# Brockaaa/scenery-insitu

Hardware: AMD Instinct MI355X
Metric: frames/sec @1920x1080 (8x512^3 volume) (higher is better)
Workload: dtype f32

## Files before the change

scenery-insitu_amd/csrc/insitu_hip.cpp:

```cpp
#include "insitu_host.h"

#include <cmath>
#include <cstdio>
#include <algorithm>
#include <cstdlib>
#include <cstring>
#include <limits>
#include <string>
#include <vector>

#pragma clang fp contract(off)

namespace {

thread_local std::string g_create_error;

size_t dtype_size(int dt) { return dt == INSITU_U8 ? 1 : (dt == INSITU_U16 ? 2 : 4); }

}

int fail(insitu_ctx* c, int code, const std::string& msg) {
    if (c) c->err = msg;
    else g_create_error = msg;
    return code;
// ... 37 lines not shown
    f.h_ctr_pending = false;
    f.h_ctr_valid = true;
    if (!c->cache_adaptive || f.h_ctr->march_rays == 0) return;
    const unsigned long long want = f.h_ctr->cache_cursor + f.h_ctr->cache_cursor / 4;
    const size_t to = std::min((size_t)want, c->cache_max_chunks);
    if (to > f.cache_chunks) f.cache_grow_to = (uint32_t)to;
}

hipError_t cache_realloc(FrameSlot& f, size_t chunks) {
    f.cache_chunks = 0;
    const hipError_t e = f.cache.try_alloc(chunks * 8);
    if (e == hipSuccess) f.cache_chunks = (uint32_t)chunks;
    return e;
}

}

int check_fault(insitu_ctx* c, FrameSlot& f) {
    cache_observe(c, f);
    if (!f.counters || !f.search_launched) return 0;
    uint32_t fault = 0;
    if (f.h_ctr_valid) fault = f.h_ctr->fault;
    else if (hipMemcpy(&fault, &f.counters->fault, sizeof fault, hipMemcpyDeviceToHost) != hipSuccess) fault = 1;
    if (fault) return fail(c, -6, "VDI search kernel exceeded its loop bound (internal error)");
    return 0;
}

namespace {

float4* cvdi_col(const insitu_ctx* c) { return c->rank == 0 ? c->d_gvdi_col : c->d_cvdi_col; }
float2* cvdi_dep(const insitu_ctx* c) { return c->rank == 0 ? c->d_gvdi_dep : c->d_cvdi_dep; }
uint16_t* cvdi_cnt(const insitu_ctx* c) { return c->rank == 0 ? c->d_gvdi_cnt : c->d_cvdi_cnt; }

void record(FrameSlot& f, FrameEvent i, hipStream_t s) {
    if (hipEventRecord(f.ev[i], s) == hipSuccess) f.ev_valid[i] = true;
}

hipError_t compact_enqueue(insitu_ctx* c, FrameSlot& f, hipStream_t s) {
    record(f, EvCompactStart, s);
    hipError_t e = hipMemsetAsync(c->d_cursor, 0, sizeof(uint32_t) * (size_t)c->N, s);
    if (e != hipSuccess) return e;
    CompactParams cp{};
    cp.col = f.vcol_send;
    cp.dep = f.vdep_send;
    cp.pend = f.seg_pending;
    cp.pend_stride = (size_t)c->W * (size_t)c->H;
    cp.W = c->W; cp.H = c->H; cp.S = c->S; cp.B = c->BV; cp.nstrips = c->N; cp.strip_w = c->strip_w;
    cp.strip_tiles = c->strip_tiles; cp.ytiles = (c->H + 7) / 8; cp.skip_d = c->rank;
    cp.blockE = c->blockE;
    cp.out_col = c->d_ccol_send;
    cp.out_dep = c->d_cdep_send;
    cp.out_meta = c->d_meta_send;
    cp.meta_bytes = c->meta_bytes;
    cp.cursor = c->d_cursor;
    e = launch_vdi_compact(cp, s);
    if (e == hipSuccess) record(f, EvCompactEnd, s);
    return e;
}

hipError_t wait_peer_reads(insitu_ctx* c, hipStream_t s) {
    if (!c->group) return hipSuccess;
    for (const insitu_ctx* q : c->group->ranks) {
        if (!q || q == c || !q->cur->ev_valid[EvPeerReadsDone]) continue;
        hipError_t e = hipStreamWaitEvent(s, q->cur->ev[EvPeerReadsDone], 0);
        if (e != hipSuccess) return e;
    }
    return hipSuccess;
}

int create_slot_events(insitu_ctx* c, FrameSlot& f) {
    for (auto& ev : f.ev)
        if (!ev && hipEventCreate(&ev) != hipSuccess) return fail(c, -3, "hipEventCreate failed");
    return 0;
}

int alloc_slot(insitu_ctx* c, FrameSlot& f, size_t chunks) {
    int rc = 0;
    if ((rc = create_slot_events(c, f))) return rc;
    const size_t sendE = (size_t)c->N * (size_t)c->BV * c->blockE;
    const size_t px = (size_t)c->BV * (size_t)c->W * (size_t)c->H;
    if ((rc = f.vcol_send.alloc(c, sendE)) || (rc = f.vdep_send.alloc(c, sendE))) return rc;
    const size_t oct = (size_t)c->BV * (size_t)c->S * (size_t)c->ncx * (size_t)c->ncy;
    if ((rc = f.octree.alloc(c, oct ? oct : 1))) return rc;
    if ((rc = f.seg_pending.alloc(c, px)) || (rc = f.seg_steps.alloc(c, sendE))) return rc;
    if (hipMemset(f.seg_pending, 0, sizeof(uint16_t) * px) != hipSuccess)
        return fail(c, -3, "hipMemset of the supersegment counts failed");
    if (c->cfg.keep_passes && (rc = f.passes.alloc(c, px))) return rc;
    if ((rc = f.counters.alloc(c, 1))) return rc;
    if (hipMemset(f.counters, 0, sizeof(GenCounters)) != hipSuccess)
        return fail(c, -3, "hipMemset of the generator counters failed");
    if (chunks == 0) return 0;
    if ((rc = f.cache.alloc(c, chunks * 8)) || (rc = f.queue.alloc(c, (size_t)c->B * (size_t)c->W * (size_t)c->H)))
        return rc;
    if (f.h_ctr.try_alloc(1) != hipSuccess) return fail(c, -5, "hipHostMalloc of the generator counters failed");
    std::memset(f.h_ctr, 0, sizeof(GenCounters));
    f.cache_chunks = (uint32_t)chunks;
    const size_t ntile = (size_t)c->B * (size_t)((c->H + 7) / 8) * (size_t)c->N * (size_t)c->strip_tiles;
    if (ntile < ((size_t)1 << 24)) {
        size_t tb = 0;
        if (sort_tiles_desc(nullptr, tb, nullptr, nullptr, nullptr, nullptr, (int)ntile, nullptr) != hipSuccess)
            return fail(c, -3, "hipcub radix sort: temporary storage query failed");
        if ((rc = f.tile_keys.alloc(c, 2 * ntile)) || (rc = f.tile_ids.alloc(c, 2 * ntile)) ||
            (rc = f.sort_tmp.alloc(c, tb + 1)))
            return rc;
        c->sort_tmp_bytes = tb;
    }
    return 0;
}

size_t padded_tiles(const insitu_ctx* c, int sup) {
    return (size_t)c->B * (size_t)((((c->H + 7) / 8) + sup - 1) / sup * sup) *
           (size_t)((c->N * c->strip_tiles + sup - 1) / sup * sup);
}

}

extern "C" {

int insitu_abi_version(void) { return INSITU_ABI_VERSION; }

int insitu_local_group_create(int nranks, insitu_local_group** out) {
    if (!out || nranks < 1 || nranks > kMaxLists) return fail(nullptr, -1, "insitu_local_group_create: bad arguments");
    *out = new insitu_local_group();
    (*out)->ranks.assign((size_t)nranks, nullptr);
    return 0;
}

void insitu_local_group_destroy(insitu_local_group* g) { delete g; }

int insitu_comm_id(void* out, size_t cap) {
    if (!out || cap < sizeof(ncclUniqueId)) return fail(nullptr, -1, "insitu_comm_id: buffer too small");
    ncclUniqueId id;
    ncclResult_t r = ncclGetUniqueId(&id);
    if (r != ncclSuccess) return fail(nullptr, -4, std::string("ncclGetUniqueId: ") + ncclGetErrorString(r));
    std::memcpy(out, &id, sizeof id);
    return 0;
}

const char* insitu_last_error(const insitu_ctx* ctx) { return ctx ? ctx->err.c_str() : g_create_error.c_str(); }

int insitu_create(const insitu_config* cfg, insitu_ctx** out) {
    if (!cfg || !out) return fail(nullptr, -1, "insitu_create: null argument");
    *out = nullptr;
    const insitu_config& k = *cfg;
    if (k.nranks < 1 || k.rank < 0 || k.rank >= k.nranks) return fail(nullptr, -1, "insitu_create: bad rank/nranks");
    if (k.width <= 0 || k.height <= 0) return fail(nullptr, -1, "insitu_create: bad window size");
    if (k.mode != INSITU_MODE_VDI && k.mode != INSITU_MODE_PLAIN) return fail(nullptr, -1, "insitu_create: bad mode");
    if (k.bricks_per_rank < 1 || k.bricks_per_rank > kMaxBricks)
        return fail(nullptr, -1, "insitu_create: bricks_per_rank must be in [1," + std::to_string(kMaxBricks) + "]");
    if (k.nranks * k.bricks_per_rank > kMaxLists)
        return fail(nullptr, -1, "insitu_create: nranks*bricks_per_rank exceeds " + std::to_string(kMaxLists));
    if (k.mode == INSITU_MODE_VDI && (k.max_supersegments < 1 || k.max_supersegments > 255))
        return fail(nullptr, -1, "insitu_create: max_supersegments must be in [1,255]");
    if (k.mode == INSITU_MODE_VDI && k.width % k.nranks != 0)
        return fail(nullptr, -1, "insitu_create: width must divide evenly into nranks screen strips");
    if (k.mode == INSITU_MODE_PLAIN && k.height % k.nranks != 0)
        return fail(nullptr, -1, "insitu_create: height (texture dim1) must divide evenly into nranks strips");
    if (k.nranks > 1 && !k.comm_id && !k.local_group)
        return fail(nullptr, -1, "insitu_create: comm_id (or local_group) required when nranks > 1");
    if (k.local_group && ((int)k.local_group->ranks.size() != k.nranks || k.local_group->ranks[k.rank]))
        return fail(nullptr, -1, "insitu_create: local_group size differs from nranks, or rank already taken");
    if (k.composite_vdi && k.mode != INSITU_MODE_VDI)
        return fail(nullptr, -1, "insitu_create: composite_vdi needs VDI mode");
    if (k.merge_bricks && k.mode != INSITU_MODE_VDI)
        return fail(nullptr, -1, "insitu_create: merge_bricks needs VDI mode");
    if (k.max_output_supersegments < 0 || k.max_output_supersegments > 255)
        return fail(nullptr, -1, "insitu_create: max_output_supersegments must be in [0,255]");
// ... 366 lines not shown
        std::memcpy(iv, cam->inv_view, sizeof iv);
        std::memcpy(ip, cam->inv_proj, sizeof ip);
    } else if (!mat4_inverse(cam->view, iv) || !mat4_inverse(cam->proj, ip)) {
        return fail(c, -1, "insitu_set_camera: view or projection matrix is singular");
    }
    mat4_mul_f(iv, ip, m->ipv);
    mat4_mul_f(cam->proj, cam->view, m->pv);
    std::memcpy(m->view, cam->view, sizeof m->view);
    m->nw = cam->nw; m->fwnw = cam->fwnw; m->tmax = cam->tmax;
    return 0;
}

void set_slot_camera(insitu_ctx* c, FrameSlot& f, const FrameCamera& m) {
    std::memcpy(f.ipv, m.ipv, sizeof f.ipv);
    std::memcpy(f.pv, m.pv, sizeof f.pv);
    std::memcpy(f.view, m.view, sizeof f.view);
    c->camera_set = true;
}

int render_check(insitu_ctx* c, const insitu_camera* cam, FrameCamera* m) {
    if (!cam) return fail(c, -1, "insitu_render: null camera");
    if (!c->d_tf) return fail(c, -1, "insitu_render: transfer function not set");
    for (int b = 0; b < c->B; ++b) {
        if (!c->bricks[b].valid) return fail(c, -1, "insitu_render: brick slot " + std::to_string(b) + " not set");
        if (c->bricks[b].dtype != c->bricks[0].dtype)
            return fail(c, -1, "insitu_render: all bricks of a rank must share one voxel type");
    }
    if (!(cam->nw > 0.0f)) return fail(c, -1, "insitu_render: nw must be > 0");
    return camera_matrices(c, cam, m);
}

struct RenderPlan {
    hipStream_t first = nullptr;
    hipStream_t search = nullptr;
    bool pipelined = false;
    unsigned long long* gate_flag = nullptr;
    unsigned long long gate_value = 0;
    hipEvent_t gate_event = nullptr;
};

int render_frame(insitu_ctx* c, FrameSlot& f, const FrameCamera& cam, const RenderPlan& plan) {
    set_slot_camera(c, f, cam);
    TransferDesc xf{c->d_tf, c->n_tf, c->d_cmap, c->n_cm, c->cmag};
    const hipStream_t ss = plan.first, sr = plan.search;
    const bool pipelined = plan.pipelined;
    HIPCHK(c, wait_peer_reads(c, ss));
    c->ingest_batch = false;
    f.pipelined = pipelined;
    if (!pipelined) record(f, EvRenderStart, ss);
    if (c->mode == INSITU_MODE_VDI) {
        const size_t oct = (size_t)c->BV * (size_t)c->S * (size_t)c->ncx * (size_t)c->ncy;
        if (oct) HIPCHK(c, hipMemsetAsync(f.octree, 0, oct * sizeof(uint32_t), ss));
        if (f.cache_grow_to > f.cache_chunks) {
            const size_t grow = f.cache_grow_to, old = f.cache_chunks;
            f.cache_grow_to = 0;
            HIPCHK(c, hipStreamSynchronize(c->stream));
            HIPCHK(c, hipStreamSynchronize(ss));
            HIPCHK(c, hipStreamSynchronize(sr));
            if (cache_realloc(f, grow) != hipSuccess) {
                const size_t keep = std::max(old, grow / 2);
                if (cache_realloc(f, keep) != hipSuccess) HIPCHK(c, cache_realloc(f, old));
                c->cache_max_chunks = f.cache_chunks;
            }
        }
        VdiGenParams p{};
        for (int b = 0; b < c->B; ++b) p.bricks[b] = brick_desc(c, c->bricks[b]);
        p.xfer = xf;
        std::memcpy(p.ipv, f.ipv, sizeof p.ipv);
        std::memcpy(p.pv, f.pv, sizeof p.pv);
        std::memcpy(p.view, f.view, sizeof p.view);
        p.nw = cam.nw;
        p.tmax = cam.tmax;
        p.W = c->W; p.H = c->H; p.S = c->S;
        p.strip_w = c->strip_w; p.strip_tiles = c->strip_tiles; p.nstrips = c->N; p.B = c->BV;
        p.nvolumes = c->BV != c->B ? c->B : 0;
        p.ytiles = (c->H + 7) / 8;
        p.color = f.vcol_send;
        p.depth = f.vdep_send;
        p.octree = f.octree;
        p.octree_stride = (size_t)c->S * (size_t)c->ncx * (size_t)c->ncy;
        p.passes = f.passes;
        p.passes_stride = (size_t)c->W * (size_t)c->H;
        p.seg_pending = f.seg_pending;
        p.seg_steps = f.seg_steps;
        p.ncx = c->ncx; p.ncy = c->ncy;
        p.interval_size = (20.0f - 0.1f) / (float)c->S;
        p.cache = f.cache;
        p.split_event = f.ev[EvSampleEnd];
        f.ev_valid[EvSampleEnd] = true;
        p.cache_chunks = f.cache_chunks;
        p.ctr = f.counters;
        p.queue = f.queue;
        p.queue_cap = (uint32_t)((size_t)c->BV * (size_t)c->W * (size_t)c->H);
        p.long_samples = (uint32_t)c->tune.long_samples;
        p.round_batch = (int)c->tune.round_batch;
        p.search_blocks = c->search_blocks;
        if (pipelined && c->tune.pipe_search_rays > 0) {
            p.search_blocks = std::min(c->search_blocks, 2 * c->num_cus);
            p.search_block_rays = (int)c->tune.pipe_search_rays;
            p.search_min_blocks = std::min(p.search_blocks, c->num_cus);
        }
        p.search_oversub = (int)(pipelined ? c->tune.pipe_oversub : c->tune.search_oversub);
        p.search_depth = (int)c->tune.search_depth;
        p.regroup = (int)c->tune.regroup;
        p.exact_search = (int)c->tune.exact_search;
        if (f.cache && (c->search_lanes_tf != c->n_tf || c->search_lanes_cm != c->n_cm)) {
            HIPCHK(c, vdi_search_resident_lanes(c->n_tf, c->n_cm, c->cfg.device, &c->search_lanes));
            c->search_lanes_tf = c->n_tf;
            c->search_lanes_cm = c->n_cm;
        }
        p.search_lanes = std::min(c->search_lanes, p.search_blocks * 256);
        if (c->tune.tile_order && f.tile_keys) {
            p.tile_keys = f.tile_keys;
            p.super_tile = (int)c->tune.super_tile;
            p.tile_len_exact = (int)c->tune.exact_tile_keys;
            p.tile_ids = f.tile_ids;
            p.sort_tmp = f.sort_tmp;
            p.sort_tmp_bytes = c->sort_tmp_bytes;
        }
        if (pipelined && f.cache && c->pipe_flag && c->pipe_trigger == 1) {
            p.pipe_flag = c->pipe_flag + f.flag_index;
            p.pipe_seq = f.flag_value + 1;
        }
        p.measure_cache = (c->cache_adaptive && !f.cache_sized && p.nvolumes == 0) ? 1 : 0;
        HIPCHK(c, launch_vdi_prepare(p, ss));
        p.prepared = 1;
        if (p.measure_cache && f.cache && p.tile_ids) {
            unsigned long long need = 0;
            HIPCHK(c, hipMemcpyAsync(&need, &f.counters->cache_need, sizeof need, hipMemcpyDeviceToHost, ss));
            HIPCHK(c, hipStreamSynchronize(ss));
            f.cache_sized = true;
            const size_t want = std::min((size_t)(need + need / 4 + 64), c->cache_max_chunks);
            if (want > f.cache_chunks) HIPCHK(c, cache_realloc(f, want));
            p.cache = f.cache;
            p.cache_chunks = f.cache_chunks;
        }
        if (pipelined) {
            if (plan.gate_flag)
                HIPCHK(c, hipStreamWaitValue64(ss, plan.gate_flag, plan.gate_value, hipStreamWaitValueGte));
            else if (plan.gate_event)
                HIPCHK(c, hipStreamWaitEvent(ss, plan.gate_event, 0));
            record(f, EvRenderStart, ss);
        }
        if (c->d_dbg && !pipelined) {
            HIPCHK(c, hipMemsetAsync(c->d_dbg, 0, c->dbg_entries * 32, ss));
            p.debug_rays = c->d_dbg;
            p.debug_cap = (uint32_t)std::min(c->dbg_entries, (size_t)0xffffffffu);
            c->dbg_pending = true;
        }
        HIPCHK(c, launch_vdi_sample(p, ss));
        if (ss != sr) HIPCHK(c, hipStreamWaitEvent(sr, f.ev[EvSampleEnd], 0));
        HIPCHK(c, launch_vdi_search(p, sr));
        f.search_launched = f.cache != nullptr;
        if (pipelined) {
            record(f, EvSearchEnd, sr);
            if (p.pipe_flag) {
                HIPCHK(c, hipStreamWriteValue64(sr, p.pipe_flag, p.pipe_seq, 0));
                f.flag_value = p.pipe_seq;
            }
        }
        HIPCHK(c, launch_vdi_finish(p, sr));
        if (f.h_ctr) {
            HIPCHK(c, hipMemcpyAsync(f.h_ctr, f.counters, sizeof(GenCounters), hipMemcpyDeviceToHost, sr));
            f.h_ctr_pending = true;
            f.h_ctr_valid = false;
        }
        if (c->N > 1 && !pipelined) HIPCHK(c, compact_enqueue(c, f, sr));
// ... 836 lines not shown
```

scenery-insitu_amd/csrc/insitu_host.h:

```cpp
#pragma once

#include "insitu_hip.h"
#include "insitu_kernels.h"

#include <hip/hip_runtime.h>
#include <rccl/rccl.h>

#include <cmath>
#include <algorithm>
#include <cstring>
#include <string>
#include <vector>

using namespace insitu;


int fail(insitu_ctx* c, int code, const std::string& msg);

template <typename T, bool Pinned = false>
class DevBuf {
public:
    DevBuf() = default;
    DevBuf(DevBuf&& o) noexcept : p_(o.p_), n_(o.n_) { o.p_ = nullptr; o.n_ = 0; }
    DevBuf& operator=(DevBuf&& o) noexcept {
// ... 51 lines not shown
    int dims[3] = {0, 0, 0};
    float im[16];
    bool valid = false;
};

inline void mat4_mul_f(const float* a, const float* b, float* out) {
    float t[16];
    for (int c = 0; c < 4; ++c) {
        const float x = b[c * 4 + 0], y = b[c * 4 + 1], z = b[c * 4 + 2], w = b[c * 4 + 3];
        for (int r = 0; r < 4; ++r)
            t[c * 4 + r] = std::fmaf(a[12 + r], w, std::fmaf(a[8 + r], z, std::fmaf(a[4 + r], y, a[r] * x)));
    }
    std::memcpy(out, t, sizeof t);
}

inline bool mat4_inverse(const float* m, float* out) {
    double a[4][8];
    for (int r = 0; r < 4; ++r) {
        for (int c = 0; c < 4; ++c) a[r][c] = (double)m[c * 4 + r];
        for (int c = 0; c < 4; ++c) a[r][4 + c] = (r == c) ? 1.0 : 0.0;
    }
    for (int col = 0; col < 4; ++col) {
        int piv = col;
        for (int r = col + 1; r < 4; ++r)
            if (std::fabs(a[r][col]) > std::fabs(a[piv][col])) piv = r;
        if (a[piv][col] == 0.0) return false;
        if (piv != col)
            for (int c = 0; c < 8; ++c) std::swap(a[piv][c], a[col][c]);
        const double inv = 1.0 / a[col][col];
        for (int c = 0; c < 8; ++c) a[col][c] *= inv;
        for (int r = 0; r < 4; ++r) {
            if (r == col) continue;
            const double f = a[r][col];
            for (int c = 0; c < 8; ++c) a[r][c] -= f * a[col][c];
        }
    }
    for (int r = 0; r < 4; ++r)
        for (int c = 0; c < 4; ++c) out[c * 4 + r] = (float)a[r][4 + c];
    return true;
}

struct insitu_local_group {
    std::vector<insitu_ctx*> ranks;
};

struct Tuning {
    long long exact_search = 0;
    long long search_depth = 0;
    long long long_samples = 384;
    long long round_batch = 28;
    long long search_oversub = 6;
    long long pipe_oversub = 3;
    long long pipe_search_rays = 2048;
    long long tile_order = 1;
    long long super_tile = 1;
    long long regroup = 1;
    long long exact_tile_keys = 0;
};

enum FrameEvent {
    EvRenderStart = 0,
    EvRenderEnd,
    EvExchangeEnd,
    EvCompositeEnd,
    EvGatherEnd,
    EvSampleEnd,
    EvCompactStart,
    EvPeerReadsDone,
    EvCountsIn,
    EvPayloadStart,
    EvImageOnHost,
    EvSlotFree,
    EvCompactEnd,
    EvSearchEnd,
    kFrameEvents
};

struct FrameSlot {
    DevBuf<float4> vcol_send;
    DevBuf<float2> vdep_send;
    DevBuf<uint32_t> octree;
    DevBuf<uint8_t> passes;
    DevBuf<uint16_t> seg_pending;
    DevBuf<uint16_t> seg_steps;
    DevBuf<GenCounters> counters;
    DevBuf<PendingRay> queue;
    DevBuf<float> cache;
    uint32_t cache_chunks = 0;
    uint32_t cache_grow_to = 0;
    bool cache_sized = false;
    PinnedBuf<GenCounters> h_ctr;
    bool h_ctr_pending = false;
    bool h_ctr_valid = false;
    bool search_launched = false;
    DevBuf<uint32_t> tile_keys;
    DevBuf<uint32_t> tile_ids;
    DevBuf<unsigned char> sort_tmp;
    float ipv[16] = {}, pv[16] = {}, view[16] = {};
    bool rendered = false, composited = false;
    bool exchanged = false;
    bool pipelined = false;
    hipStream_t search_stream = nullptr;
    int flag_index = 0;
    unsigned long long flag_value = 0;
    hipEvent_t ev[kFrameEvents] = {};
    bool ev_valid[kFrameEvents] = {};
};

struct ViewState {
    DevBuf<float4> col;
    DevBuf<float2> dep;
    DevBuf<uint8_t> cnt, tmax;
    ViewVdi vdi{};
    float pv_g[16] = {};
    bool bound = false;
    DevBuf<float4> out_color;
    DevBuf<uint32_t> out_image;
    int out_w = 0, out_h = 0;
    hipStream_t stream = nullptr;
    hipEvent_t ev0 = nullptr, ev1 = nullptr;
    float ms = 0.0f;
    long long skip = 1;
    long long compact_next = 0;
    DevBuf<uint16_t> loc;
    bool counted = false;
    unsigned long long pk_E = 0;
    DevBuf<uint32_t> pk_bstat;
    DevBuf<unsigned long long> pk_boff;
    DevBuf<PackTotals> pk_totals;
    PinnedBuf<PackTotals> h_totals;
    DevBuf<unsigned char> pk_stage;
    float ms_pack = 0.0f;
    DevBuf<MergeTotals> mg_totals;
    PinnedBuf<MergeTotals> h_mg_totals;
    long long overlaps = 0;
    float ms_bind = 0.0f;
    DevBuf<unsigned char> ps_stage;
    DevBuf<unsigned char> ps_index;
    PinnedBuf<PackTotals> h_ps_totals;
    DevBuf<unsigned char> gm_ctl;
    PinnedBuf<unsigned char> h_gm_ctl;
    struct GatherOffer {
        enum { None, Made, Withdrawn } state = None;
        unsigned char header[128] = {};
        const uint8_t* cnt = nullptr;
        const float2* dep = nullptr;
        const void* col = nullptr;
        hipEvent_t ev = nullptr;
    } offer;
};

struct insitu_ctx {
    insitu_config cfg{};
    insitu_local_group* group = nullptr;
    int W = 0, H = 0, S = 0, N = 1, rank = 0, B = 1, V = 1, mode = INSITU_MODE_VDI;
    int BV = 1;
    int strip_w = 0, strip_tiles = 0, rows = 0, ncx = 0, ncy = 0;
    size_t blockE = 0;
    size_t plainBlock = 0;
    size_t stripPx = 0;
    hipStream_t stream = nullptr;
    bool own_stream = false;
    ncclComm_t comm = nullptr;
    std::vector<Brick> bricks;
    DevBuf<float> d_tf;
    DevBuf<float> d_cmap;
    int n_tf = 0, n_cm = 0;
// ... 103 lines not shown
```

scenery-insitu_amd/csrc/insitu_kernels.h:

```cpp
#pragma once
#include <hip/hip_runtime.h>
#include <stddef.h>
#include <stdint.h>

namespace insitu {

enum VoxelType { VOX_U8 = 0, VOX_U16 = 1, VOX_F32 = 2 };

struct BrickDesc {
    const void* data;
    int dtype;
    int nx, ny, nz;
    int nbx, nby, nbz;
    float im[16];
    float conv_k;
    float conv_off;
};

struct TransferDesc {
    const float* tf;
    int n_tf;
    const float* cmap;
    int n_cm;
    float cmag;
};

constexpr int kMaxBricks = 8;

struct PendingRay {
    uint32_t pix;
    uint32_t b;
    uint32_t chunk;
    uint32_t n;
    float step_first;
    uint32_t last_final;
    float low, high, mid;
    uint32_t iter_found;
    float seg_low[2], seg_high[2];
    uint32_t n_high;
    uint32_t nsteps;
};

struct GenCounters {
    unsigned long long cache_cursor;
    uint32_t queue_count;
    uint32_t queue_head;
    uint32_t fault;
    uint32_t queue_short;
    uint32_t march_rays;
    uint32_t cap_overflow;
    unsigned long long cache_need;
    uint32_t regroups;
    unsigned long long* pipe_flag;
    unsigned long long pipe_seq;
};

struct VdiGenParams {
    BrickDesc bricks[kMaxBricks];
    int nvolumes;
    size_t octree_stride;
    size_t passes_stride;
    TransferDesc xfer;
    float ipv[16];
    float pv[16];
    float view[16];
    float nw, tmax;
    int W, H, S;
    int strip_w, strip_tiles, nstrips, B;
    int ytiles;
    float4* color;
    float2* depth;
    uint32_t* octree;
    uint8_t* passes;
    uint16_t* seg_pending;
    uint16_t* seg_steps;
    float* cache;
    uint32_t cache_chunks;
    GenCounters* ctr;
    PendingRay* queue;
    uint32_t queue_cap;
    uint32_t long_samples;
    int round_batch;
    int search_blocks;
    int search_block_rays;
    int search_min_blocks;
    int search_lanes;
    int search_oversub;
    int search_depth;
    int regroup;
    hipEvent_t split_event;
    int exact_search;
    unsigned long long* debug_rays;
    uint32_t debug_cap;
    int ncx, ncy;
    float interval_size;
    uint32_t* tile_keys;
    uint32_t* tile_ids;
    void* sort_tmp;
    size_t sort_tmp_bytes;
    int super_tile;
    int tile_len_exact;
    int prepared;
    int measure_cache;
    unsigned long long* pipe_flag;
    unsigned long long pipe_seq;
};

constexpr uint32_t kPendingCount = 0xffu;
constexpr uint32_t kPendingDeferred = 0x100u;
constexpr uint32_t kPendingCounted = 0x200u;

struct PlainGenParams {
    BrickDesc bricks[kMaxBricks];
    TransferDesc xfer;
    float ipv[16];
    float nw, fwnw, tmax;
    int dim0, dim1;
    int rows;
    int nstrips, B;
    uint32_t* color;
    uint32_t* depth;
};

constexpr int kMaxLists = 32;

struct VdiList {
    const float4* col;
    const float2* dep;
    const uint16_t* cnt16;
    int cnt_pitch, cnt_x0;
    const uint8_t* cnt8;
    const uint32_t* toff;
};

struct FlattenParams {
    VdiList lists[kMaxLists];
    int V, S, H, W;
    int strip_w, strip_tiles, x_offset;
    float ipv[16];
    uint32_t* out;
};

struct CompositeParams {
    VdiList lists[kMaxLists];
    int V, S, S_out, H, W;
    int strip_w, strip_tiles, x_offset;
    float ipv[16];
    float4* out_color;
    float2* out_depth;
    uint16_t* out_count;
    int ndc_local;
    uint8_t* passes;
    float4* seq;
    unsigned long long* seq_cursor;
    unsigned long long seq_cap;
    int exact;
};
constexpr int kCompEntryF4 = 2;
// ... 150 lines not shown
```

scenery-insitu_amd/csrc/vdi_generate.hip:

```cpp
#include "insitu_sampling.h"
#include "insitu_filter.h"

#pragma clang fp contract(off)

namespace insitu {

__device__ __forceinline__ int find_z_interval_view(float z_view, float interval_size, int ncz) {
    float dist_from_front = __builtin_fabsf(z_view - (-1.0f * 0.1f));
    float q = __builtin_floorf(dist_from_front / interval_size);
    if (!(q < (float)ncz)) return ncz;
    return (int)q;
}

__host__ __device__ __forceinline__ size_t chunk_off(uint32_t c) { return (size_t)c * 64u; }

__host__ __device__ __forceinline__ size_t mslot_off(uint32_t c) { return (size_t)(c / 2u) * 128u + (c % 2u); }

struct RayOut {
    float4* color;
    float2* depth;
    uint32_t slot_stride;
};

__device__ __forceinline__ void octree_range(const VdiGenParams& P, float uvx, float uvy, float start, float end,
// ... 1029 lines not shown
                              lane, b, tile);
}

constexpr int kSpecFrom = 8;
constexpr int kSpecFromGroup = 7;
constexpr int kSearchMinWaves = 3;
constexpr int kMaxSearchDepth = 6;
constexpr int kMaxRegroupDepth = 4;

constexpr int kP1LdsFloats = 512 * (kSpecLevels + 1) + 8 * 256;
__host__ __device__ __forceinline__ size_t sample_lds_bytes(int n_tf, int n_cm) {
    return lut_lds_bytes(n_tf, n_cm) + (size_t)kP1LdsFloats * 4;
}
__host__ __device__ __forceinline__ size_t merge_lds_bytes(int n_tf, int n_cm) {
    return lut_lds_bytes(n_tf, n_cm) + (size_t)(512 * (kSpecLevels + 1) + 20 * 256) * 4;
}

__host__ __device__ __forceinline__ size_t search_lds_bytes(int n_tf, int n_cm) {
    return lut_lds_bytes(n_tf, n_cm) + 4 * 256 * 16 + 256 * 4 + 2 * 16 + 256 * 4 + 256 * 8 + 256 * 8;
}

constexpr int kGroupBatch = 6;
constexpr float kDeepWindow = 3e-3f;
__device__ __forceinline__ Thr search_thr(float t_sq, float c, const Search& q) {
    Thr r = make_thr(t_sq, c);
    if (!q.found && q.high - q.low < kDeepWindow) {
        r.hi = __builtin_fmaxf(r.hi, make_thr(sq_threshold(q.high), c).hi);
        r.lo = __builtin_fminf(r.lo, make_thr(sq_threshold(q.low), c).lo);
    }
    return r;
}

template <bool FILTERED, bool MERGED>
__device__ __forceinline__ void search_loop(const VdiGenParams& P, float4* smem) {
    float4* s_cm = smem;
    float* s_tf = reinterpret_cast<float*>(smem + lut_cm_slots(P.xfer.n_cm));
    float4* s_c0 = smem + lut_cm_slots(P.xfer.n_cm) + lut_tf_slots(P.xfer.n_tf);
    float4* s_w0 = s_c0 + 256;
    float4* s_res = s_c0 + 512;
    float4* s_iv = s_c0 + 768;
    int* s_nh = reinterpret_cast<int*>(s_c0 + 1024);
    float4* s_pv = s_c0 + 1024 + 64;
    uint32_t* s_dbg_slot = reinterpret_cast<uint32_t*>(s_c0 + 1024 + 66);
    unsigned long long* s_dbg_t0 = reinterpret_cast<unsigned long long*>(s_c0 + 1024 + 66 + 64);
    uint2* s_s0 = reinterpret_cast<uint2*>(s_c0 + 1024 + 66 + 64 + 128);
    const int tid = threadIdx.x;
    const int lane = threadIdx.x & 63;
    GenCounters* const ctr = P.ctr;
    const uint32_t qlong = ctr->queue_count;
    const uint32_t qlen = qlong + ctr->queue_short;
    if (qlen == 0u) return;
    unsigned long long lanes = (unsigned long long)P.search_lanes;
    if (P.search_block_rays > 0) {
        uint32_t active = (qlen + (uint32_t)P.search_block_rays - 1u) / (uint32_t)P.search_block_rays;
        active = active < (uint32_t)P.search_min_blocks ? (uint32_t)P.search_min_blocks : active;
        if (blockIdx.x >= active) return;
        const unsigned long long al = (unsigned long long)active * 256ull;
        lanes = al < lanes ? al : lanes;
    }
    int d = 1;
    const unsigned long long cap = lanes * (unsigned long long)P.search_oversub;
    if ((unsigned long long)qlen * 15ull <= cap) d = 4;
    else if ((unsigned long long)qlen * 7ull <= cap) d = 3;
    else if ((unsigned long long)qlen * 3ull <= cap) d = 2;
    if (P.search_depth > 0) d = P.search_depth;
    int G = (1 << d) - 1;
    int node = lane % G, gbase = lane - node;
    bool member = lane < (64 / G) * G;
    bool leader_lane = member && node == 0;
    int spec_from = G == 1 ? kSpecFrom : kSpecFromGroup;
    int home = tid;

    const int S = P.S;
    const int delta = (int)__builtin_floorf(0.15f * (float)S);
    float nw = P.nw;
    asm volatile("" : "+v"(nw));
    bool active = false, drained = false;
    uint32_t pix = 0, bslot = 0;
    uint32_t chunk = 0;
    uint32_t nsteps = 0;
    float step_first = 0.0f;
    bool last_final = false;
    f4 wfront{}, wback{};
    size_t e0 = 0;
    const size_t slot_stride = (size_t)P.H * 8;
    Search q{};
    Thr th{};
    SegState st;
    st.reset();
    int nseg = 0, k = 0, n = 0, nchunks = 1, pre_chunk = 0;
    uint32_t cur_step = 0;
    uint2 s4{}, ps4{};
    float stp = 0.0f;
    float4 c4{}, w4{};
    float4 pc4{}, pw4{};
    auto ndc_of = [](float t) { return t; };
    auto take = [&](uint32_t r, uint32_t slot) {
        const PendingRay pr = P.queue[slot];
        home = (tid - lane) + gbase;
        pix = pr.pix;
        bslot = pr.b;
        chunk = pr.chunk;
        nsteps = pr.nsteps;
        step_first = pr.step_first;
        last_final = pr.last_final != 0u;
        const int gy = (int)(pix / (uint32_t)P.W), gx = (int)(pix - (uint32_t)gy * (uint32_t)P.W);
        {
            Ray R;
            ray_dirs(P, gx, gy, R);
            wfront = R.wfront;
            wback = R.wback;
        }
        e0 = (size_t)(ray_out(P, gx, gy, (int)bslot).color - P.color);
        const float4* cbase = reinterpret_cast<const float4*>(P.cache) + 2 * (size_t)chunk;
        n = (int)pr.n;
        nchunks = (n + 3) >> 2;
        q = Search{pr.low, pr.high, pr.mid, (int)(pr.iter_found & 0xffu), (pr.iter_found & 0x100u) != 0,
                   false, false};
        q.written = q.found;
        s_iv[home] = make_float4(pr.seg_low[0], pr.seg_low[1], pr.seg_high[0], pr.seg_high[1]);
        s_nh[home] = (int)pr.n_high;
        th = search_thr(sq_threshold(q.found ? q.mid : tree_threshold(q.low, q.high, q.mid, node)), P.xfer.cmag, q);
        st.reset();
        k = 0;
        nseg = 0;
        stp = step_first;
        s_c0[home] = cbase[0];
        s_w0[home] = cbase[1];
        if constexpr (MERGED) s_s0[home] = *reinterpret_cast<const uint2*>(cbase + 2);
        active = true;
        if (P.debug_rays) {
            s_dbg_slot[home] = r;
            s_dbg_t0[home] = wall_clock64();
        }
    };
    const unsigned long long t_end = wall_clock64() + 1000000000ull;
    uint32_t trips = 0u;
    for (;;) {
        if ((++trips & 255u) == 0u && wall_clock64() > t_end) {
            if (lane == 0) atomicOr(&ctr->fault, 1u);
            break;
        }
        const unsigned long long idle = __ballot(!active && leader_lane);
        if (idle != 0ull && !drained) {
            const int first = __builtin_ctzll(idle);
            const uint32_t cnt = (uint32_t)__popcll(idle);
            uint32_t base = 0;
            if (lane == first) base = atomicAdd(&ctr->queue_head, cnt);
            base = __shfl(base, first);
            if (base + cnt >= qlen) {
                if (base < qlen && lane == first) {
                    unsigned long long* const flag = ctr->pipe_flag;
                    if (flag) __hip_atomic_store(flag, ctr->pipe_seq, __ATOMIC_RELEASE, __HIP_MEMORY_SCOPE_SYSTEM);
                }
                drained = true;
            }
            uint32_t r = base + (uint32_t)__popcll(idle & ((1ull << lane) - 1ull));
            r = __shfl(r, gbase);
            if (!active && member && r < qlen) take(r, r < qlong ? r : P.queue_cap - 1u - (r - qlong));
        }
        if (__ballot(active) == 0ull) {
            if (drained) break;
            continue;
        }
        bool hold = false;
        if (P.regroup && drained) {
            const unsigned long long lead = __ballot(active && leader_lane);
            const int R = __popcll(lead);
            int dn = d;
            while (dn < kMaxRegroupDepth && R * ((1 << (dn + 1)) - 1) <= 64) dn++;
            if (dn > d) {
                if (__ballot(active && k != 0) == 0ull) {
                    const int Gn = (1 << dn) - 1;
                    const int g = lane / Gn, nd = lane - g * Gn;
                    unsigned long long m = lead;
                    for (int i = 0; i < g && m != 0ull; ++i) m &= m - 1ull;
                    const int src = m != 0ull ? __builtin_ctzll(m) : 0;
                    pix = (uint32_t)__shfl((int)pix, src);
                    bslot = (uint32_t)__shfl((int)bslot, src);
                    chunk = (uint32_t)__shfl((int)chunk, src);
                    nsteps = (uint32_t)__shfl((int)nsteps, src);
                    step_first = __shfl(step_first, src);
                    last_final = __shfl((int)last_final, src) != 0;
                    n = __shfl(n, src);
                    q.low = __shfl(q.low, src);
                    q.high = __shfl(q.high, src);
                    q.mid = __shfl(q.mid, src);
                    q.iter = __shfl(q.iter, src);
                    q.found = __shfl((int)q.found, src) != 0;
                    q.written = __shfl((int)q.written, src) != 0;
                    home = __shfl(home, src);
                    wfront = f4{__shfl(wfront.x, src), __shfl(wfront.y, src), __shfl(wfront.z, src), __shfl(wfront.w, src)};
                    wback = f4{__shfl(wback.x, src), __shfl(wback.y, src), __shfl(wback.z, src), __shfl(wback.w, src)};
                    e0 = (size_t)(uint32_t)__shfl((int)(uint32_t)e0, src) |
                         ((size_t)(uint32_t)__shfl((int)(uint32_t)(e0 >> 32), src) << 32);
                    if (lane == 0) atomicAdd(&ctr->regroups, 1u);
                    d = dn;
                    G = Gn;
                    node = nd;
                    gbase = g * Gn;
                    member = g < R;
                    leader_lane = member && nd == 0;
                    spec_from = kSpecFromGroup;
                    active = member;
                    nchunks = (n + 3) >> 2;
                    if (active) {
                        th = search_thr(sq_threshold(q.found ? q.mid : tree_threshold(q.low, q.high, q.mid, node)),
                                        P.xfer.cmag, q);
                        st.reset();
                        k = 0;
                        nseg = 0;
                        stp = step_first;
                    }
                } else {
                    hold = active && k == 0;
                }
            }
        }
        if (active && k < n && !hold) {
            if (k == 0) {
                c4 = s_c0[home];
                w4 = s_w0[home];
                pre_chunk = 0;
                if constexpr (MERGED) {
                    s4 = s_s0[home];
                    cur_step = s4.x & 0xffffu;
                }
            } else {
                c4 = pc4;
                w4 = pw4;
                if constexpr (MERGED) s4 = ps4;
            }
            pre_chunk++;
            if (pre_chunk < nchunks) {
                const float4* nx = reinterpret_cast<const float4*>(P.cache) + 2 * (size_t)chunk +
                                   (MERGED ? 4 * mslot_off((uint32_t)pre_chunk) : 2 * chunk_off((uint32_t)pre_chunk));
                pc4 = nx[0];
                pw4 = nx[1];
                if constexpr (MERGED) ps4 = *reinterpret_cast<const uint2*>(nx + 2);
            }
            const f4 x0 = classify_sample(c4.x, s_tf, P.xfer.n_tf, s_cm, P.xfer.n_cm);
            const f4 x1 = classify_sample(c4.y, s_tf, P.xfer.n_tf, s_cm, P.xfer.n_cm);
            const f4 x2 = classify_sample(c4.z, s_tf, P.xfer.n_tf, s_cm, P.xfer.n_cm);
            const f4 x3 = classify_sample(c4.w, s_tf, P.xfer.n_tf, s_cm, P.xfer.n_cm);
            const bool write = q.written && node == 0;
            const bool store = (q.written || q.iter + 1 >= spec_from) && node == 0;
            auto emit = [&](float s0, float e1, const f4& cv, int steps) {
                if (store) {
                    if (nseg < S) {
                        const size_t e = e0 + (size_t)nseg * slot_stride;
                        P.color[e] = make_float4(cv.x, cv.y, cv.z, cv.w);
                        P.depth[e] = make_float2(s0, e1);
                        P.seg_steps[e] = (uint16_t)steps;
                    } else if (write) {
                        const int gy = (int)(pix / (uint32_t)P.W), gx = (int)(pix - (uint32_t)gy * (uint32_t)P.W);
                        Ray R;
                        ray_dirs(P, gx, gy, R);
                        octree_update(P, P.octree + (size_t)bslot * P.octree_stride, R.uvx, R.uvy,
                                      ndc_at_rows(s_pv, wfront, wback, s0), ndc_at_rows(s_pv, wfront, wback, e1), R.cx,
                                      R.cy);
                    }
                    nseg++;
                }
            };
            if constexpr (FILTERED) {
#define INSITU_REPLAY_SEL(XV, WV, SI)                                                                          \
    {                                                                                                          \
        const bool on = k < n;                                                                                 \
        bool last;                                                                                             \
        if constexpr (MERGED) {                                                                                \
            const uint32_t si = (SI);                                                                          \
            last = si + 1u == nsteps;                                                                          \
            if (store && on)                                                                                   \
                while (cur_step < si) {                 \
                    stp = stp + nw;                                                                            \
                    cur_step++;                                                                                \
                }                                                                                              \
        } else {                                                                                               \
            last = last_final && k == n - 1;                                                                   \
        }                                                                                                      \
        seg_sample_sel(st, (XV), (WV), stp, on, last, th, wfront, wback, nw, emit, store);                     \
        if constexpr (!MERGED) stp = stp + nw;                                                                 \
        k = on ? ((!q.written && st.nterm > S) ? n : k + 1) : k;                                               \
    }
                INSITU_REPLAY_SEL(x0, w4.x, s4.x & 0xffffu)
                INSITU_REPLAY_SEL(x1, w4.y, s4.x >> 16)
                INSITU_REPLAY_SEL(x2, w4.z, s4.y & 0xffffu)
                INSITU_REPLAY_SEL(x3, w4.w, s4.y >> 16)
#undef INSITU_REPLAY_SEL
            } else {
#define INSITU_REPLAY(XV, WV, SI)                                                                              \
    if (k < n) {                                                                                               \
        bool last;                                                                                             \
        if constexpr (MERGED) {                                                                                \
            const uint32_t si = (SI);                                                                          \
            last = si + 1u == nsteps;                                                                       \
            if (store)                                                                                         \
                while (cur_step < si) {                 \
                    stp = stp + nw;                                                                            \
                    cur_step++;                                                                                \
                }                                                                                              \
        } else {                                                                                               \
            last = last_final && k == n - 1;                                                                \
        }                                                                                                      \
        seg_sample<true, true>(st, (XV), (WV), stp, ndc_of, last, th, wfront, wback, nw, emit);                \
        if constexpr (!MERGED) stp = stp + nw;                                                                 \
        k = (!q.written && st.nterm > S) ? n : k + 1;                                                          \
    }
            INSITU_REPLAY(x0, w4.x, s4.x & 0xffffu)
            INSITU_REPLAY(x1, w4.y, s4.x >> 16)
            INSITU_REPLAY(x2, w4.z, s4.y & 0xffffu)
            INSITU_REPLAY(x3, w4.w, s4.y >> 16)
#undef INSITU_REPLAY
            }
        }
        const unsigned long long fin = __ballot(active && k >= n);
        const unsigned long long gmask = ((1ull << G) - 1ull) << gbase;
        const bool round_end = active && (fin & gmask) == gmask;
        const unsigned long long re = __ballot(round_end);
        if (re == 0ull) continue;
        if (__popcll(re) < (G == 1 ? P.round_batch : kGroupBatch) && __ballot(active && k < n && !hold) != 0ull) continue;
        if (round_end) {
            float lo = st.lo, hi = st.hi;
            if constexpr (FILTERED) {
                lo = __builtin_fmaxf(lo, seg_lo_bound(st.lo_a, P.xfer.cmag));
                hi = __builtin_fminf(hi, seg_hi_bound(st.hi_a, P.xfer.cmag));
            }
            s_res[tid] = make_float4(__int_as_float(st.nterm), lo, hi, 0.0f);
        }
        __builtin_amdgcn_fence(__ATOMIC_RELEASE, "wavefront");
        __builtin_amdgcn_wave_barrier();
        __builtin_amdgcn_fence(__ATOMIC_ACQUIRE, "wavefront");
        if (round_end) {
            bool done = q.written;
            if (done) {
                q.iter++;
            } else {
                float4 iv = s_iv[home];
                int n_high = s_nh[home];
                int at = 0;
                bool stored = false;
                for (int lvl = 0; lvl < d; ++lvl) {
                    const float4 res = s_res[tid - node + at];
                    const int cnt_here = __float_as_int(res.x);
                    q.iter++;
                    const bool more = cnt_here > S;
                    const bool narrow = __builtin_fabsf(q.high - q.low) < 0.000001f;
                    search_step(q, cnt_here, S, delta, res.y, res.z, iv, n_high);
                    stored = lvl == 0 && q.found && !narrow && q.iter >= spec_from;
                    if (q.found || q.iter >= 64) break;
                    at = more ? 2 * at + 1 : 2 * at + 2;
                }
                if (q.iter < 64) free_walk(q, iv, n_high, S, delta);
                s_iv[home] = iv;
                s_nh[home] = n_high;
                if (q.iter + 1 > 64) {
                    q.iter++;
                    nseg = 0;
                    done = true;
                } else if (stored) {
                    q.iter++;
                    done = true;
                } else {
                    if (q.found) q.written = true;
                    th = search_thr(sq_threshold(q.found ? q.mid : tree_threshold(q.low, q.high, q.mid, node)), P.xfer.cmag, q);
                    st.reset();
                    k = 0;
                    nseg = 0;
                    stp = step_first;
                }
            }
            if (done) {
                if (node == 0) {
                    if (P.passes) P.passes[(size_t)bslot * P.passes_stride + pix] = (uint8_t)q.iter;
                    P.seg_pending[(size_t)bslot * P.passes_stride + pix] = (uint16_t)((nseg < S ? nseg : S) | kPendingDeferred);
                }
                active = false;
            }
        }
        if (round_end && !active && P.debug_rays && node == 0) {
            unsigned long long* e = P.debug_rays + 4 * (size_t)s_dbg_slot[home];
            e[0] = s_dbg_t0[home];
            e[1] = wall_clock64();
            e[2] = (unsigned long long)q.iter | ((unsigned long long)n << 8) | ((unsigned long long)G << 24);
            e[3] = pix | ((unsigned long long)bslot << 32);
        }
    }
}

__device__ __forceinline__ void stage_pv_rows(const VdiGenParams& P, float4* smem) {
    float4* s_pv = smem + lut_cm_slots(P.xfer.n_cm) + lut_tf_slots(P.xfer.n_tf) + 1024 + 64;
    if (threadIdx.x == 0) {
        s_pv[0] = make_float4(P.pv[2], P.pv[6], P.pv[10], P.pv[14]);
        s_pv[1] = make_float4(P.pv[3], P.pv[7], P.pv[11], P.pv[15]);
    }
    __syncthreads();
}

template <bool FILTERED, bool MERGED>
__global__ __launch_bounds__(256, kSearchMinWaves) void vdi_search_kernel(const VdiGenParams P) {
    extern __shared__ __attribute__((aligned(16))) float4 smem[];
    stage_luts(P.xfer, smem, reinterpret_cast<float*>(smem + lut_cm_slots(P.xfer.n_cm)));
    stage_pv_rows(P, smem);
    search_loop<FILTERED, MERGED>(P, smem);
}

constexpr int kFinishMinBlocks = 1;
__global__ __launch_bounds__(256, kFinishMinBlocks) void vdi_finish_kernel(const VdiGenParams P) {
    extern __shared__ uint32_t s_hist[];
    const int wave = threadIdx.x >> 6, lane = threadIdx.x & 63;
    uint32_t* hist = s_hist + wave * P.S;
    for (int j = lane; j < P.S; j += 64) hist[j] = 0u;
    const int b = (int)blockIdx.y;
    const int tile = (int)blockIdx.x * 4 + wave;
    const int yt = tile % P.ytiles, ct = tile / P.ytiles;
    const int d = ct / P.strip_tiles, xt = ct % P.strip_tiles;
    const int xl = xt * 8 + (lane & 7), gy = yt * 8 + (lane >> 3);
    const bool valid = d < P.nstrips && xl < P.strip_w && gy < P.H;
    const int gx = d * P.strip_w + xl;
    const uint32_t pend = valid ? P.seg_pending[(size_t)b * P.passes_stride + (size_t)gy * (size_t)P.W + (size_t)gx] : 0u;
    const bool deferred = (pend & kPendingDeferred) != 0u;
    const bool count_cells = (pend & kPendingCounted) == 0u;
    const int cnt = (deferred || count_cells) ? (int)(pend & kPendingCount) : 0;
    const unsigned long long act = __ballot(cnt > 0);
    if (act == 0ull) return;
    Ray R{};
    ray_dirs(P, gx, gy, R);
    const bool in_grid = R.cx >= 0 && R.cx < P.ncx && R.cy >= 0 && R.cy < P.ncy;
    const int cell = R.cy * P.ncx + R.cx;
    const int first = __builtin_ctzll(act);
    const int cell0 = __shfl(cell, first);
    const bool uniform = __ballot(cnt > 0 && (cell != cell0 || !in_grid)) == 0ull;
    uint32_t* oct = P.octree + (size_t)b * P.octree_stride;
    __builtin_amdgcn_wave_barrier();
    if (cnt > 0) {
        const RayOut o = ray_out(P, gx, gy, b);
        const size_t e0 = (size_t)(o.color - P.color);
        for (int i0 = 0; i0 < cnt; i0 += 4) {
            float2 se[4];
            float4 cv[4];
            uint16_t st[4];
#pragma unroll
            for (int u = 0; u < 4; ++u) {
                const int i = i0 + u < cnt ? i0 + u : cnt - 1;
                const size_t e = e0 + (size_t)i * o.slot_stride;
                se[u] = P.depth[e];
                if (deferred) {
                    cv[u] = P.color[e];
                    st[u] = P.seg_steps[e];
                }
            }
#pragma unroll
            for (int u = 0; u < 4; ++u) {
                if (i0 + u >= cnt) break;
                const size_t e = e0 + (size_t)(i0 + u) * o.slot_stride;
                float2 d = se[u];
                if (deferred) {
                    d = make_float2(ndc_at(P, R.wfront, R.wback, d.x), ndc_at(P, R.wfront, R.wback, d.y));
                    P.depth[e] = d;
                    const f4 a = exact_adjusted(f4{cv[u].x, cv[u].y, cv[u].z, cv[u].w}, (int)st[u], R.wfront, R.wback, P.nw);
                    P.color[e] = make_float4(a.x, a.y, a.z, a.w);
                }
                if (count_cells && uniform) {
                    int sc, ec;
                    octree_range(P, R.uvx, R.uvy, d.x, d.y, sc, ec);
                    for (int j = sc; j <= ec && j < P.S; ++j) atomicAdd(&hist[j], 1u);
                } else if (count_cells) {
                    octree_update(P, oct, R.uvx, R.uvy, d.x, d.y, R.cx, R.cy);
                }
            }
        }
    }
    __builtin_amdgcn_fence(__ATOMIC_RELEASE, "wavefront");
    __builtin_amdgcn_wave_barrier();
    __builtin_amdgcn_fence(__ATOMIC_ACQUIRE, "wavefront");
    if (uniform) {
        for (int j = lane; j < P.S; j += 64) {
            const uint32_t v = hist[j];
            if (v) atomicAdd(&oct[(uint32_t)j * (uint32_t)(P.ncx * P.ncy) + (uint32_t)cell0], v);
        }
    }
}

hipError_t launch_vdi_finish(const VdiGenParams& p, hipStream_t s) {
    if (!p.seg_pending || !p.seg_steps) return hipErrorInvalidValue;
    const int tiles = p.ytiles * p.nstrips * p.strip_tiles;
    hipLaunchKernelGGL(vdi_finish_kernel, dim3((tiles + 3) / 4, p.B), dim3(256), 4 * sizeof(uint32_t) * p.S, s, p);
    return hipGetLastError();
}

size_t vdi_generator_lds_bytes(int n_tf, int n_cm) {
    const size_t a = sample_lds_bytes(n_tf, n_cm), b = merge_lds_bytes(n_tf, n_cm), c = search_lds_bytes(n_tf, n_cm);
    return a > b ? (a > c ? a : c) : (b > c ? b : c);
}

hipError_t vdi_search_resident_lanes(int n_tf, int n_cm, int device, int* lanes) {
    int blocks_per_cu = 1 << 30, cus = 0;
    hipError_t e = hipSuccess;
    const size_t lds = search_lds_bytes(n_tf, n_cm);
    for (const void* k : {reinterpret_cast<const void*>(vdi_search_kernel<true, false>),
                          reinterpret_cast<const void*>(vdi_search_kernel<false, false>),
                          reinterpret_cast<const void*>(vdi_search_kernel<true, true>),
                          reinterpret_cast<const void*>(vdi_search_kernel<false, true>)}) {
        int n = 0;
        e = hipOccupancyMaxActiveBlocksPerMultiprocessor(&n, k, 256, lds);
        if (e != hipSuccess) return e;
        blocks_per_cu = n < blocks_per_cu ? n : blocks_per_cu;
    }
    if (e == hipSuccess) e = hipDeviceGetAttribute(&cus, hipDeviceAttributeMultiprocessorCount, device);
    if (e != hipSuccess) return e;
    *lanes = blocks_per_cu * cus * 256;
    return hipSuccess;
}

hipError_t launch_vdi_prepare(const VdiGenParams& p, hipStream_t s) {
    const int tiles = p.ytiles * p.nstrips * p.strip_tiles;
    hipError_t e = hipMemsetAsync(p.ctr, 0, sizeof(GenCounters), s);
    if (e == hipSuccess && p.pipe_flag) {
        e = hipStreamWriteValue64(s, &p.ctr->pipe_flag, (uint64_t)(uintptr_t)p.pipe_flag, 0);
        if (e == hipSuccess) e = hipStreamWriteValue64(s, &p.ctr->pipe_seq, p.pipe_seq, 0);
    }
    if (e != hipSuccess || !p.tile_ids) return e;
    const int n = p.B * tiles;
    const int sup = p.super_tile, sup2 = sup * sup;
    if (sup != 1 && sup != 2 && sup != 4) return hipErrorInvalidValue;
    const int nsuper = ((p.nstrips * p.strip_tiles + sup - 1) / sup) * ((p.ytiles + sup - 1) / sup);
    const int wpb = sup2 > 4 ? sup2 : 4;
    const int spb = wpb / sup2;
    if (sup == 1 && !p.measure_cache && !p.tile_len_exact)
        hipLaunchKernelGGL(vdi_tile_len_sub_kernel, dim3((tiles + 15) / 16, p.B), dim3(256), 0, s, p);
    else
        hipLaunchKernelGGL(vdi_tile_len_kernel, dim3((nsuper + spb - 1) / spb, p.B), dim3(64 * wpb), 0, s, p);
    size_t tb = p.sort_tmp_bytes;
    return sort_tiles_desc(p.sort_tmp, tb, p.tile_keys, p.tile_keys + n, p.tile_ids, p.tile_ids + n, n, s);
}

hipError_t launch_vdi_sample(const VdiGenParams& p, hipStream_t s) {
    const int tiles = p.ytiles * p.nstrips * p.strip_tiles;
    const dim3 grid((tiles + 3) / 4, p.B);
    const size_t lds = sample_lds_bytes(p.xfer.n_tf, p.xfer.n_cm);
    if (p.B < 1 || p.B > kMaxBricks || !p.seg_pending || !p.seg_steps || !p.ctr) return hipErrorInvalidValue;
    for (int b = 1; b < p.B; ++b)
        if (p.bricks[b].dtype != p.bricks[0].dtype) return hipErrorInvalidValue;
    if (p.cache) {
        if (!p.queue || p.search_lanes <= 0 || p.search_depth < 0 || p.search_depth > kMaxSearchDepth)
            return hipErrorInvalidValue;
    }
    hipError_t e = hipSuccess;
    if (!p.prepared) {
        e = launch_vdi_prepare(p, s);
        if (e != hipSuccess) return e;
    }
    const bool f = !p.exact_search;
    if (p.nvolumes > 0) {
        if (p.B != 1 || p.nvolumes > kMaxBricks) return hipErrorInvalidValue;
        for (int b = 1; b < p.nvolumes; ++b)
            if (p.bricks[b].dtype != p.bricks[0].dtype) return hipErrorInvalidValue;
        const dim3 mgrid((tiles + 3) / 4);
        const size_t lds_merge = merge_lds_bytes(p.xfer.n_tf, p.xfer.n_cm);
        switch (p.bricks[0].dtype) {
        case VOX_U8:
            if (f) hipLaunchKernelGGL((vdi_merge_kernel<VOX_U8, true>), mgrid, dim3(256), lds_merge, s, p);
            else hipLaunchKernelGGL((vdi_merge_kernel<VOX_U8, false>), mgrid, dim3(256), lds_merge, s, p);
            break;
        case VOX_U16:
            if (f) hipLaunchKernelGGL((vdi_merge_kernel<VOX_U16, true>), mgrid, dim3(256), lds_merge, s, p);
            else hipLaunchKernelGGL((vdi_merge_kernel<VOX_U16, false>), mgrid, dim3(256), lds_merge, s, p);
            break;
        case VOX_F32:
            if (f) hipLaunchKernelGGL((vdi_merge_kernel<VOX_F32, true>), mgrid, dim3(256), lds_merge, s, p);
            else hipLaunchKernelGGL((vdi_merge_kernel<VOX_F32, false>), mgrid, dim3(256), lds_merge, s, p);
            break;
        default: return hipErrorInvalidValue;
        }
    } else {
        dim3 sgrid = grid;
        if (p.tile_ids) sgrid = dim3((p.B * tiles + 3) / 4, 1);
        switch (p.bricks[0].dtype) {
        case VOX_U8:
            if (f) hipLaunchKernelGGL((vdi_sample_kernel<VOX_U8, true>), sgrid, dim3(256), lds, s, p);
            else hipLaunchKernelGGL((vdi_sample_kernel<VOX_U8, false>), sgrid, dim3(256), lds, s, p);
            break;
        case VOX_U16:
            if (f) hipLaunchKernelGGL((vdi_sample_kernel<VOX_U16, true>), sgrid, dim3(256), lds, s, p);
            else hipLaunchKernelGGL((vdi_sample_kernel<VOX_U16, false>), sgrid, dim3(256), lds, s, p);
            break;
        case VOX_F32:
            if (f) hipLaunchKernelGGL((vdi_sample_kernel<VOX_F32, true>), sgrid, dim3(256), lds, s, p);
            else hipLaunchKernelGGL((vdi_sample_kernel<VOX_F32, false>), sgrid, dim3(256), lds, s, p);
            break;
        default: return hipErrorInvalidValue;
        }
    }
    e = hipGetLastError();
    if (e == hipSuccess && p.split_event) e = hipEventRecord(p.split_event, s);
    return e;
}

hipError_t launch_vdi_search(const VdiGenParams& p, hipStream_t s) {
    if (!p.cache) return hipSuccess;
    const bool f = !p.exact_search;
    const size_t lds_search = search_lds_bytes(p.xfer.n_tf, p.xfer.n_cm);
    if (p.nvolumes > 0) {
        if (f) hipLaunchKernelGGL((vdi_search_kernel<true, true>), dim3(p.search_blocks), dim3(256), lds_search, s, p);
        else hipLaunchKernelGGL((vdi_search_kernel<false, true>), dim3(p.search_blocks), dim3(256), lds_search, s, p);
        return hipGetLastError();
    }
    if (f) hipLaunchKernelGGL((vdi_search_kernel<true, false>), dim3(p.search_blocks), dim3(256), lds_search, s, p);
    else hipLaunchKernelGGL((vdi_search_kernel<false, false>), dim3(p.search_blocks), dim3(256), lds_search, s, p);
    return hipGetLastError();
}

hipError_t launch_vdi_generate(const VdiGenParams& p, hipStream_t s) {
    hipError_t e = launch_vdi_sample(p, s);
    return e == hipSuccess ? launch_vdi_search(p, s) : e;
}

}
```

Baseline: 68.19.

## Pack deferred segment color, depth and step count into one 32-byte record

Deferred supersegment output used to go to three separate arrays (color float4, depth float2, steps uint16), which meant three scattered stores per emitted segment and three loads in the finish kernel. It now goes to a single 32-byte SegRecord per slot, written with two 16-byte vector stores through a running pointer and read back with two vector loads. This cuts the number of memory transactions per segment. In exchange the scratch buffer gets larger, because the uint16 steps field is widened and padded, and the non-deferred path still reads depth from the old array.

```diff
diff --git a/scenery-insitu_amd/csrc/insitu_hip.cpp b/scenery-insitu_amd/csrc/insitu_hip.cpp
--- a/scenery-insitu_amd/csrc/insitu_hip.cpp
+++ b/scenery-insitu_amd/csrc/insitu_hip.cpp
@@ -143,7 +143,7 @@
     if ((rc = f.vcol_send.alloc(c, sendE)) || (rc = f.vdep_send.alloc(c, sendE))) return rc;
     const size_t oct = (size_t)c->BV * (size_t)c->S * (size_t)c->ncx * (size_t)c->ncy;
     if ((rc = f.octree.alloc(c, oct ? oct : 1))) return rc;
-    if ((rc = f.seg_pending.alloc(c, px)) || (rc = f.seg_steps.alloc(c, sendE))) return rc;
+    if ((rc = f.seg_pending.alloc(c, px)) || (rc = f.seg_rec.alloc(c, sendE))) return rc;
     if (hipMemset(f.seg_pending, 0, sizeof(uint16_t) * px) != hipSuccess)
         return fail(c, -3, "hipMemset of the supersegment counts failed");
     if (c->cfg.keep_passes && (rc = f.passes.alloc(c, px))) return rc;
@@ -676,7 +676,7 @@
         p.passes = f.passes;
         p.passes_stride = (size_t)c->W * (size_t)c->H;
         p.seg_pending = f.seg_pending;
-        p.seg_steps = f.seg_steps;
+        p.seg_rec = f.seg_rec;
         p.ncx = c->ncx; p.ncy = c->ncy;
         p.interval_size = (20.0f - 0.1f) / (float)c->S;
         p.cache = f.cache;
diff --git a/scenery-insitu_amd/csrc/insitu_host.h b/scenery-insitu_amd/csrc/insitu_host.h
--- a/scenery-insitu_amd/csrc/insitu_host.h
+++ b/scenery-insitu_amd/csrc/insitu_host.h
@@ -157,7 +157,7 @@
     DevBuf<uint32_t> octree;
     DevBuf<uint8_t> passes;
     DevBuf<uint16_t> seg_pending;
-    DevBuf<uint16_t> seg_steps;
+    DevBuf<SegRecord> seg_rec;
     DevBuf<GenCounters> counters;
     DevBuf<PendingRay> queue;
     DevBuf<float> cache;
diff --git a/scenery-insitu_amd/csrc/insitu_kernels.h b/scenery-insitu_amd/csrc/insitu_kernels.h
--- a/scenery-insitu_amd/csrc/insitu_kernels.h
+++ b/scenery-insitu_amd/csrc/insitu_kernels.h
@@ -54,6 +54,14 @@
     unsigned long long* pipe_flag;
     unsigned long long pipe_seq;
 };
+
+struct alignas(32) SegRecord {
+    float4 curV;
+    float s0, e1;
+    uint32_t steps;
+    uint32_t unused;
+};
+static_assert(sizeof(SegRecord) == 32, "SegRecord is one 32-byte sector");
 
 struct VdiGenParams {
     BrickDesc bricks[kMaxBricks];
@@ -73,7 +81,7 @@
     uint32_t* octree;
     uint8_t* passes;
     uint16_t* seg_pending;
-    uint16_t* seg_steps;
+    SegRecord* seg_rec;
     float* cache;
     uint32_t cache_chunks;
     GenCounters* ctr;
diff --git a/scenery-insitu_amd/csrc/vdi_generate.hip b/scenery-insitu_amd/csrc/vdi_generate.hip
--- a/scenery-insitu_amd/csrc/vdi_generate.hip
+++ b/scenery-insitu_amd/csrc/vdi_generate.hip
@@ -1135,8 +1135,8 @@
     float step_first = 0.0f;
     bool last_final = false;
     f4 wfront{}, wback{};
-    size_t e0 = 0;
-    const size_t slot_stride = (size_t)P.H * 8;
+    uintptr_t rec = 0;
+    const uint32_t rec_stride = (uint32_t)P.H * 8u * (uint32_t)sizeof(SegRecord);
     Search q{};
     Thr th{};
     SegState st;
@@ -1164,7 +1164,7 @@
             wfront = R.wfront;
             wback = R.wback;
         }
-        e0 = (size_t)(ray_out(P, gx, gy, (int)bslot).color - P.color);
+        rec = reinterpret_cast<uintptr_t>(P.seg_rec + (ray_out(P, gx, gy, (int)bslot).color - P.color));
         const float4* cbase = reinterpret_cast<const float4*>(P.cache) + 2 * (size_t)chunk;
         n = (int)pr.n;
         nchunks = (n + 3) >> 2;
@@ -1245,8 +1245,8 @@
                     home = __shfl(home, src);
                     wfront = f4{__shfl(wfront.x, src), __shfl(wfront.y, src), __shfl(wfront.z, src), __shfl(wfront.w, src)};
                     wback = f4{__shfl(wback.x, src), __shfl(wback.y, src), __shfl(wback.z, src), __shfl(wback.w, src)};
-                    e0 = (size_t)(uint32_t)__shfl((int)(uint32_t)e0, src) |
-                         ((size_t)(uint32_t)__shfl((int)(uint32_t)(e0 >> 32), src) << 32);
+                    rec = (uintptr_t)(uint32_t)__shfl((int)(uint32_t)rec, src) |
+                          ((uintptr_t)(uint32_t)__shfl((int)(uint32_t)(rec >> 32), src) << 32);
                     if (lane == 0) atomicAdd(&ctr->regroups, 1u);
                     d = dn;
                     G = Gn;
@@ -1301,10 +1301,11 @@
             auto emit = [&](float s0, float e1, const f4& cv, int steps) {
                 if (store) {
                     if (nseg < S) {
-                        const size_t e = e0 + (size_t)nseg * slot_stride;
-                        P.color[e] = make_float4(cv.x, cv.y, cv.z, cv.w);
-                        P.depth[e] = make_float2(s0, e1);
-                        P.seg_steps[e] = (uint16_t)steps;
+                        typedef float v4f __attribute__((ext_vector_type(4)));
+                        typedef __attribute__((address_space(1))) v4f global_v4f;
+                        global_v4f* const r = reinterpret_cast<global_v4f*>(rec);
+                        r[0] = v4f{cv.x, cv.y, cv.z, cv.w};
+                        r[1] = v4f{s0, e1, __uint_as_float((uint32_t)steps), 0.0f};
                     } else if (write) {
                         const int gy = (int)(pix / (uint32_t)P.W), gx = (int)(pix - (uint32_t)gy * (uint32_t)P.W);
                         Ray R;
@@ -1314,6 +1315,7 @@
                                       R.cy);
                     }
                     nseg++;
+                    rec += rec_stride;
                 }
             };
             if constexpr (FILTERED) {
@@ -1419,6 +1421,7 @@
                     th = search_thr(sq_threshold(q.found ? q.mid : tree_threshold(q.low, q.high, q.mid, node)), P.xfer.cmag, q);
                     st.reset();
                     k = 0;
+                    rec -= (uintptr_t)(uint32_t)nseg * rec_stride;
                     nseg = 0;
                     stp = step_first;
                 }
@@ -1492,15 +1495,19 @@
         for (int i0 = 0; i0 < cnt; i0 += 4) {
             float2 se[4];
             float4 cv[4];
-            uint16_t st[4];
+            uint32_t st[4];
 #pragma unroll
             for (int u = 0; u < 4; ++u) {
                 const int i = i0 + u < cnt ? i0 + u : cnt - 1;
                 const size_t e = e0 + (size_t)i * o.slot_stride;
-                se[u] = P.depth[e];
                 if (deferred) {
-                    cv[u] = P.color[e];
-                    st[u] = P.seg_steps[e];
+                    const float4* const r = reinterpret_cast<const float4*>(P.seg_rec + e);
+                    cv[u] = r[0];
+                    const float4 t = r[1];
+                    se[u] = make_float2(t.x, t.y);
+                    st[u] = __float_as_uint(t.z);
+                } else {
+                    se[u] = P.depth[e];
                 }
             }
 #pragma unroll
@@ -1536,7 +1543,7 @@
 }
 
 hipError_t launch_vdi_finish(const VdiGenParams& p, hipStream_t s) {
-    if (!p.seg_pending || !p.seg_steps) return hipErrorInvalidValue;
+    if (!p.seg_pending || !p.seg_rec) return hipErrorInvalidValue;
     const int tiles = p.ytiles * p.nstrips * p.strip_tiles;
     hipLaunchKernelGGL(vdi_finish_kernel, dim3((tiles + 3) / 4, p.B), dim3(256), 4 * sizeof(uint32_t) * p.S, s, p);
     return hipGetLastError();
@@ -1592,7 +1599,7 @@
     const int tiles = p.ytiles * p.nstrips * p.strip_tiles;
     const dim3 grid((tiles + 3) / 4, p.B);
     const size_t lds = sample_lds_bytes(p.xfer.n_tf, p.xfer.n_cm);
-    if (p.B < 1 || p.B > kMaxBricks || !p.seg_pending || !p.seg_steps || !p.ctr) return hipErrorInvalidValue;
+    if (p.B < 1 || p.B > kMaxBricks || !p.seg_pending || !p.seg_rec || !p.ctr) return hipErrorInvalidValue;
     for (int b = 1; b < p.B; ++b)
         if (p.bricks[b].dtype != p.bricks[0].dtype) return hipErrorInvalidValue;
     if (p.cache) {
```

Result: faster. 71.00 (median of 6 runs) (+4.1%).
